# arindamrc/video_analytics

Hardware: AMD Instinct MI355X
Metric: clips/sec (224x224, RGB+10-flow two-stream) (higher is better)
Workload: dtype f32; 1 GPU; two-stream 224x224, 10-frame TV-L1 flow stack (5 scales x 5 warps x 300 its, fixed), VGG-16 spatial+temporal, batch=32 per GPU; global_batch=32, block_iters=0, tvl1_math=exact, flow_streams=2, batches_in_flight=1, tvl1_params=, tvl1_hip_blob=20e9f45376b19dd960a619139aafc0e8722a8659, parallelism=clips sharded x1, finite=True

## Files before the change

video_analytics_amd/csrc/tvl1.hip:

```cpp
#include "va_internal.h"
#include <cmath>
#include <algorithm>
#include <cstdlib>
#include <cstring>
#include <utility>
#include <type_traits>

namespace {

constexpr int kMaxScales = 16;
constexpr int kMaxRadius = 8;
constexpr int kNF_STATE = 6;
constexpr int kNF_RO = 4;

struct Taps {
    float g[2 * kMaxRadius + 1];
    int R;
};

__device__ __forceinline__ int d_min(int a, int b) { return a < b ? a : b; }
__device__ __forceinline__ int d_max(int a, int b) { return a > b ? a : b; }

__device__ __forceinline__ int pslot(int x, int perm) { return perm ? ((x & ~3) | ((x & 1) << 1) | ((x >> 1) & 1)) : x; }

__device__ __forceinline__ float bilinear(const float* __restrict__ img, int w, int h, int pitch, float x, float y, int perm = 0)
{
    x = fminf(fmaxf(x, 0.0f), (float)(w - 1));
    y = fminf(fmaxf(y, 0.0f), (float)(h - 1));
    const int x0 = (int)x, y0 = (int)y;
    const int x1 = d_min(x0 + 1, w - 1), y1 = d_min(y0 + 1, h - 1);
    const float ax = x - (float)x0, ay = y - (float)y0;
    const int s0 = pslot(x0, perm), s1 = pslot(x1, perm);
    const float a = img[y0 * pitch + s0], b = img[y0 * pitch + s1];
    const float c = img[y1 * pitch + s0], d = img[y1 * pitch + s1];
    const float top = fmaf(ax, b - a, a);
    const float bot = fmaf(ax, d - c, c);
    return fmaf(ay, bot - top, top);
}


template <typename T>
__global__ void k_frames_to_level0(const T* __restrict__ frames, float* __restrict__ pyr0, int w, int h, int pitch,
                                   size_t plane)
{
    const int f = blockIdx.y;
    const int idx = blockIdx.x * blockDim.x + threadIdx.x;
    if (idx >= w * h) return;
    const int y = idx / w, x = idx - y * w;
    pyr0[(size_t)f * 3 * plane + (size_t)y * pitch + x] = (float)frames[(size_t)f * w * h + idx];
}

template <bool VERT>
__global__ void k_gauss(const float* __restrict__ src, size_t src_fstride, float* __restrict__ dst, size_t dst_fstride,
                        int w, int h, int pitch, Taps t)
{
    const int f = blockIdx.y;
    const int idx = blockIdx.x * blockDim.x + threadIdx.x;
    if (idx >= w * h) return;
    const int y = idx / w, x = idx - y * w;
    const float* s = src + (size_t)f * src_fstride;
    const int R = t.R;
    float acc;
    if (VERT) {
        acc = t.g[0] * s[d_max(y - R, 0) * pitch + x];
        for (int k = -R + 1; k <= R; ++k) acc = fmaf(t.g[k + R], s[d_min(d_max(y + k, 0), h - 1) * pitch + x], acc);
    } else {
        acc = t.g[0] * s[y * pitch + d_max(x - R, 0)];
// ... 61 lines not shown
    }
    float r[3];
#pragma unroll
    for (int k = 0; k < 3; ++k) {
        const float top = fmaf(ax, b[k] - a[k], a[k]);
        const float bot = fmaf(ax, d[k] - c[k], c[k]);
        r[k] = fmaf(ay, bot - top, top);
    }
    v0 = r[0];
    v1 = r[1];
    v2 = r[2];
}

__global__ void k_warp(const float* __restrict__ pyr, size_t plane, int w, int h, int pitch, int fps,
                       const float* __restrict__ stA, const float* __restrict__ stB, const int* __restrict__ sel, int cur,
                       int* __restrict__ base, float* __restrict__ ro, int pair0, int perm)
{
    unsigned lid = blockIdx.y * gridDim.x + blockIdx.x;
    {
        const unsigned nb = gridDim.x * gridDim.y, q = nb / 8, r = nb % 8, xcd = lid % 8, kk = lid / 8;
        lid = (xcd < r ? xcd * (q + 1) : r * (q + 1) + (xcd - r) * q) + kk;
    }
    const int pair = pair0 + (int)(lid / gridDim.x);
    const int idx = (int)(lid % gridDim.x) * blockDim.x + threadIdx.x;
    const int which = sel ? sel[pair] : cur;
    if (base && idx == 0) base[pair] = which;
    const bool active = idx < w * h;
    const int y = active ? idx / w : 0, x = active ? idx - y * w : 0;
    const int seq = pair / (fps - 1), k = pair - seq * (fps - 1);
    const int f0 = seq * fps + k;
    const float* I0 = pyr + (size_t)f0 * 3 * plane;
    const float* I1 = pyr + (size_t)(f0 + 1) * 3 * plane;
    const float* st = (which ? stB : stA) + (size_t)pair * kNF_STATE * plane;
    const size_t o = (size_t)y * pitch + x, op = (size_t)y * pitch + pslot(x, perm);
    const float u1 = active ? st[op] : 0.0f, u2 = active ? st[plane + op] : 0.0f;
    float Iw, Iwx, Iwy;
    bilinear3_shfl(I1, plane, w, h, pitch, (float)x + u1, (float)y + u2, active, Iw, Iwx, Iwy);
    if (!active) return;
    const float grad = fmaf(Iwy, Iwy, Iwx * Iwx);
    float* r = ro + (size_t)pair * kNF_RO * plane;
    r[op] = Iwx;
    r[plane + op] = Iwy;
    r[2 * plane + op] = fmaf(-Iwy, u2, fmaf(-Iwx, u1, Iw - I0[o]));
    r[3 * plane + op] = grad < 1e-10f ? 0.0f : 1.0f / grad;
}

__global__ void k_upsample(const float* __restrict__ stA, const float* __restrict__ stB, const int* __restrict__ sel,
                           int cur, int cw, int ch, int cpitch, size_t cplane, float* __restrict__ tmp, int fw, int fh,
                           int fpitch, size_t fplane, float inv_step, int cperm)
{
    const int pair = blockIdx.y;
    const int idx = blockIdx.x * blockDim.x + threadIdx.x;
    if (idx >= fw * fh) return;
    const int which = sel ? sel[pair] : cur;
    const float* src = (which ? stB : stA) + (size_t)pair * kNF_STATE * cplane;
    float* dst = tmp + (size_t)pair * 2 * fplane;
    const int y = idx / fw, x = idx - y * fw;
    const float rx = (float)cw / (float)fw, ry = (float)ch / (float)fh;
    const size_t o = (size_t)y * fpitch + x;
    dst[o] = bilinear(src, cw, ch, cpitch, (float)x * rx, (float)y * ry, cperm) * inv_step;
    dst[fplane + o] = bilinear(src + cplane, cw, ch, cpitch, (float)x * rx, (float)y * ry, cperm) * inv_step;
}

__global__ void k_level_init(const float* __restrict__ tmp, float* __restrict__ st0, int w, int h, int pitch, size_t plane, int perm)
{
    const int pair = blockIdx.y;
    const int idx = blockIdx.x * blockDim.x + threadIdx.x;
    if (idx >= pitch * h) return;
    const int y = idx / pitch, x = idx - y * pitch;
    const size_t o = (size_t)y * pitch + x, op = (size_t)y * pitch + pslot(x, perm);
    const float* t = tmp + (size_t)pair * 2 * plane;
    float* dst = st0 + (size_t)pair * kNF_STATE * plane;
    dst[op] = x < w ? t[o] : 0.0f;
    dst[plane + op] = x < w ? t[plane + o] : 0.0f;
    dst[2 * plane + op] = 0.0f;
    dst[3 * plane + op] = 0.0f;
    dst[4 * plane + op] = 0.0f;
    dst[5 * plane + op] = 0.0f;
}

__global__ void k_zero_pad(float* __restrict__ buf, int nf, int w, int h, int pitch, size_t plane, int perm)
{
    const int pair = blockIdx.y, pw = pitch - w;
    const int idx = blockIdx.x * blockDim.x + threadIdx.x;
    if (idx >= pw * h * nf) return;
    const int f = idx / (pw * h), r = idx - f * pw * h, y = r / pw, x = w + r - y * pw;
    buf[((size_t)pair * nf + f) * plane + (size_t)y * pitch + pslot(x, perm)] = 0.0f;
}

__global__ void k_flow_out(const float* __restrict__ stA, const float* __restrict__ stB, const int* __restrict__ sel,
                           int cur, int w, int h, int pitch, size_t plane, float* __restrict__ flow, int perm)
{
    const int pair = blockIdx.y;
    const int idx = blockIdx.x * blockDim.x + threadIdx.x;
    if (idx >= w * h) return;
    const int which = sel ? sel[pair] : cur;
    const float* st = (which ? stB : stA) + (size_t)pair * kNF_STATE * plane;
    const int y = idx / w, x = idx - y * w;
    flow[((size_t)pair * 2) * w * h + idx] = st[(size_t)y * pitch + pslot(x, perm)];
    flow[((size_t)pair * 2 + 1) * w * h + idx] = st[plane + (size_t)y * pitch + pslot(x, perm)];
}

__global__ void k_flow_to_stack(const float* __restrict__ flow, float* __restrict__ stack, size_t n, float bound,
                                float mean, float stdv)
{
    const size_t i = (size_t)blockIdx.x * blockDim.x + threadIdx.x;
    if (i >= n) return;
    const float t = (255.0f * (flow[i] + bound)) / (2.0f * bound);
    const float q = rintf(fminf(fmaxf(t, 0.0f), 255.0f));
    stack[i] = (q / 255.0f - mean) / stdv;
}


struct IterArgs {
    const float* ro;
    const float* stA;
    const float* stB;
    float* outA;
    float* outB;
    const int* base;
    int* sel;
    unsigned long long* err;
    unsigned long long qthr;
    size_t plane;
    int cur;
    int w, h, pitch;
    int K;
    int ntx, nty, HX;
    int it, iters;
    int rev;
    int pair0;
    float l_t, taut, theta;
};

__device__ __forceinline__ float dpp_from_left(float v)
{
    return __builtin_bit_cast(float, __builtin_amdgcn_update_dpp(0, __builtin_bit_cast(int, v), 0x138, 0xf, 0xf, true));
}
__device__ __forceinline__ float dpp_from_right(float v)
{
    return __builtin_bit_cast(float, __builtin_amdgcn_update_dpp(0, __builtin_bit_cast(int, v), 0x130, 0xf, 0xf, true));
}

typedef float f2 __attribute__((ext_vector_type(2)));
#ifndef VA_REV
#define VA_REV 1
#endif
#ifndef VA_STREAM_QUEUE_DEFAULT
#define VA_STREAM_QUEUE_DEFAULT 0
#endif
#ifndef VA_STREAM4_DEFAULT
#define VA_STREAM4_DEFAULT 0
#endif
#ifndef VA_STREAM_UNROLL2
#define VA_STREAM_UNROLL2 1
#endif
#ifndef VA_CHUNK
#define VA_CHUNK 1
#endif
#ifndef VA_TIMING_SKIP
#define VA_TIMING_SKIP 0
#endif
#ifndef VA_CHUNK_MB
#define VA_CHUNK_MB 150.0
#endif

__device__ __forceinline__ f2 pk_fma(f2 a, f2 b, f2 c) { return __builtin_elementwise_fma(a, b, c); }
__device__ __forceinline__ float sub_s(float a, float b)
{
    float r;
    asm("v_sub_f32 %0, %1, %2" : "=v"(r) : "v"(a), "v"(b));
    return r;
}
__device__ __forceinline__ f2 splat(float v) { return f2{v, v}; }

constexpr float kSqrtReg = 7.888609052210118e-31f;
__device__ __forceinline__ f2 sqrt_exact_pk(f2 s)
// ... 449 lines not shown
    typedef StreamShape<KH, NCH> SH;
    constexpr int NP = R::NP, NT = R::NT, SW = 64 * PPL, KC = SH::KC;
    constexpr int NRING = stream_ring_rows<KH, NWV, NCH>() > 0 ? stream_ring_rows<KH, NWV, NCH>() : 1;
    __shared__ f2 ringP_[SUBS][NRING][kNF_RO][NP][64];
    __shared__ float ringT_[SUBS][NRING][kNF_RO][NT ? 64 : 1];
    __shared__ f2 ifaceP_[SUBS][NWV > 1 ? NWV - 1 : 1][2][kNF_STATE][NP][64];
    __shared__ float ifaceT_[SUBS][NWV > 1 ? NWV - 1 : 1][2][kNF_STATE][NT ? 64 : 1];
    auto& ringP = ringP_[sub];
    auto& ringT = ringT_[sub];
    auto& ifaceP = ifaceP_[sub];
    auto& ifaceT = ifaceT_[sub];

    const int sx = job % a.nsx, ch = job / a.nsx;
    const int w = a.w, h = a.h, pitch = a.pitch;
    const int lane = threadIdx.x & 63;
    const int wv = NWV == 1 ? 0 : role >= 0 ? role : __builtin_amdgcn_readfirstlane((int)(threadIdx.x >> 6));
    const int ox = sx * (SW - 2 * a.HX);
    const int vx0 = ox + (sx > 0 ? a.HX : 0), vx1 = (sx == a.nsx - 1) ? pitch : ox + SW - a.HX;
    const int x0 = ox + PPL * (half ? (lane & 31) : lane);
    const bool colok = x0 < pitch && !(half == 2 && lane >= 32);
    const bool stok = colok && x0 >= vx0 && x0 < vx1;
    const int a0 = ch * a.R, b0 = d_min(h, a0 + a.R);
    const int ys = d_max(0, a0 - K), ye = d_min(h, b0 + K);

    const int planeb = (int)(a.plane * sizeof(float)), pitchb = pitch * (int)sizeof(float);
    const int npr = half == 1 ? 2 : 1;
    const __amdgpu_buffer_rsrc_t rs_ro = __builtin_amdgcn_make_buffer_rsrc(
        const_cast<float*>(a.ro + (size_t)pair * kNF_RO * a.plane), 0, npr * kNF_RO * planeb, 0x00020000);
    const __amdgpu_buffer_rsrc_t rs_in = __builtin_amdgcn_make_buffer_rsrc(
        const_cast<float*>(sin_all + (size_t)pair * kNF_STATE * a.plane), 0, npr * kNF_STATE * planeb, 0x00020000);
    const __amdgpu_buffer_rsrc_t rs_out = __builtin_amdgcn_make_buffer_rsrc(sout_all + (size_t)pair * kNF_STATE * a.plane, 0,
                                                                           npr * kNF_STATE * planeb, 0x00020000);
    const bool second = half == 1 && lane >= 32;
    const int loff = colok ? x0 * (int)sizeof(float) + (second ? kNF_STATE * planeb : 0) : 0;
    const int loff_ro = colok ? x0 * (int)sizeof(float) + (second ? kNF_RO * planeb : 0) : 0;

    R mx;
    mx.t = 0.0f;
#pragma clang loop unroll(full)
    for (int i = 0; i < PPL; ++i) row_set(mx, i, x0 + i < w - 1 ? 1.0f : 0.0f);
    const float l_t = a.l_t, taut = a.taut, theta = a.theta;
    const R zero = row_splat<PPL>(0.0f), one = row_splat<PPL>(1.0f);

    auto ring_put = [&](int slot, int f, const R& v) __attribute__((always_inline)) {
#pragma clang loop unroll(full)
        for (int j = 0; j < NP; ++j) ringP[slot][f][j][lane] = v.p[j];
        if constexpr (NT) ringT[slot][f][lane] = v.t;
    };
    auto ring_get = [&](int slot, int f) __attribute__((always_inline)) -> R {
        R v;
#pragma clang loop unroll(full)
        for (int j = 0; j < NP; ++j) v.p[j] = ringP[slot][f][j][lane];
        v.t = 0.0f;
        if constexpr (NT) v.t = ringT[slot][f][lane];
        return v;
    };
    auto if_put = [&](int wb, int b, int f, const R& v) __attribute__((always_inline)) {
#pragma clang loop unroll(full)
        for (int j = 0; j < NP; ++j) ifaceP[wb][b][f][j][lane] = v.p[j];
        if constexpr (NT) ifaceT[wb][b][f][lane] = v.t;
    };
    auto if_get = [&](int wb, int b, int f) __attribute__((always_inline)) -> R {
        R v;
#pragma clang loop unroll(full)
        for (int j = 0; j < NP; ++j) v.p[j] = ifaceP[wb][b][f][j][lane];
        v.t = 0.0f;
        if constexpr (NT) v.t = ifaceT[wb][b][f][lane];
        return v;
    };

    for (int r = wv; r < NRING; r += NWV)
#pragma clang loop unroll(full)
        for (int f = 0; f < kNF_RO; ++f) ring_put(r, f, zero);
    if constexpr (NWV > 1) {
        if (wv < NWV - 1)
#pragma clang loop unroll(full)
            for (int f = 0; f < kNF_STATE; ++f) {
                if_put(wv, 0, f, zero);
                if_put(wv, 1, f, zero);
            }
        __syncthreads();
    }

    auto ld = [&](const __amdgpu_buffer_rsrc_t& r, int f, int y) -> R { return row_load<PPL>(r, loff, f * planeb + y * pitchb); };
    auto ld_ro = [&](int f, int y) -> R { return row_load<PPL>(rs_ro, loff_ro, f * planeb + y * pitchb); };
    auto st = [&](const R& v, int f, int y) { row_store<PPL>(v, rs_out, loff, f * planeb + y * pitchb); };

    const int nsteps = active ? b0 - ys + K + (NWV * NCH - 1) : 0;

    auto run = [&](auto wave_tag) __attribute__((always_inline)) {
        constexpr int W = decltype(wave_tag)::value;
        constexpr bool FIRST = W == 0, LAST = W == NWV - 1;
        constexpr int G0 = W * KH, LAG = W * SH::SPAN;

        R P11[KH], P12[KH], P21[KH], P22[KH], U1[KH], U2[KH];
#pragma clang loop unroll(full)
        for (int t = 0; t < KH; ++t) P11[t] = P12[t] = P21[t] = P22[t] = U1[t] = U2[t] = zero;
        SR latch[NCH > 1 ? NCH - 1 : 1];
#pragma clang loop unroll(full)
        for (int c = 0; c < (NCH > 1 ? NCH - 1 : 1); ++c) latch[c] = SR{zero, zero, zero, zero, zero, zero};
        R nst[kNF_STATE], nro[kNF_RO], rprev[kNF_RO] = {zero, zero, zero, zero};
        constexpr bool KEEP = LAST && stream_keep_last<KH, NWV, NCH>();
        R keep[kNF_RO] = {zero, zero, zero, zero};
#pragma clang loop unroll(full)
        for (int f = 0; f < kNF_STATE; ++f) nst[f] = FIRST ? ld(rs_in, f, ys) : zero;
#pragma clang loop unroll(full)
        for (int f = 0; f < kNF_RO; ++f) nro[f] = FIRST ? ld_ro(f, ys) : zero;

        auto level = [&](int t, SR& c, const R& wx, const R& wy, const R& rc, const R& ig, const float my, auto my1_tag) __attribute__((always_inline)) {
            constexpr bool MY1 = decltype(my1_tag)::value;
            const R dx11 = r_diff_back(c.p11), dx21 = r_diff_back(c.p21);
            const R div1 = r_add(dx11, r_sub(c.p12, P12[t]));
            const R div2 = r_add(dx21, r_sub(c.p22, P22[t]));
            const R rho = r_fma(wy, c.u2, r_fma(wx, c.u1, rc));
            const R tt = r_negmul(rho, ig);
            const R fi = r_med3(tt, -l_t, l_t);
            const R v1 = r_fma(fi, wx, c.u1);
            const R v2 = r_fma(fi, wy, c.u2);
            const R n1 = r_fma_s(theta, div1, v1);
            const R n2 = r_fma_s(theta, div2, v2);
            const R d1x = r_diff_fwd(U1[t]), d2x = r_diff_fwd(U2[t]);
            const R u1x = r_mul(d1x, mx), u1y = MY1 ? r_sub(n1, U1[t]) : r_mul_s(r_sub(n1, U1[t]), my);
            const R u2x = r_mul(d2x, mx), u2y = MY1 ? r_sub(n2, U2[t]) : r_mul_s(r_sub(n2, U2[t]), my);
            const R s1 = r_fma(u1y, u1y, r_fma_c(u1x, u1x, kSqrtReg));
            const R s2 = r_fma(u2y, u2y, r_fma_c(u2x, u2x, kSqrtReg));
            const R d1 = r_fma_s(taut, r_sqrt<PPL, FAST>(s1), one);
            const R d2 = r_fma_s(taut, r_sqrt<PPL, FAST>(s2), one);
            R q1, q2;
            if constexpr (FAST) {
                q1 = r_rcp<PPL, true>(d1);
                q2 = r_rcp<PPL, true>(d2);
            } else {
                const R rinv = r_rcp<PPL, false>(r_mul(d1, d2));
                q1 = r_mul(d2, rinv);
                q2 = r_mul(d1, rinv);
            }
            const R o11 = r_mul(r_fma_s(taut, u1x, P11[t]), q1);
            const R o12 = r_mul(r_fma_s(taut, u1y, P12[t]), q1);
            const R o21 = r_mul(r_fma_s(taut, u2x, P21[t]), q2);
            const R o22 = r_mul(r_fma_s(taut, u2y, P22[t]), q2);
            const R ou1 = U1[t], ou2 = U2[t];
            P11[t] = c.p11;
            P12[t] = c.p12;
            P21[t] = c.p21;
            P22[t] = c.p22;
            U1[t] = n1;
            U2[t] = n2;
            c.u1 = ou1;
            c.u2 = ou2;
            c.p11 = o11;
            c.p12 = o12;
            c.p21 = o21;
            c.p22 = o22;
        };

        auto step = [&](const int s, auto steady_tag) __attribute__((always_inline)) {
            constexpr bool STEADY = decltype(steady_tag)::value;
            const int s0 = s % NRING;
            SR cc[NCH];
            R r0[kNF_RO] = {zero, zero, zero, zero};
            if constexpr (FIRST) {
                cc[0] = SR{nst[0], nst[1], nst[2], nst[3], nst[4], nst[5]};
#pragma clang loop unroll(full)
                for (int f = 0; f < kNF_RO; ++f) r0[f] = nro[f];
                const int rn = d_min(ys + s + 1, ye - 1);
                if (!(STEADY && (VA_TIMING_SKIP & 2))) {
#pragma clang loop unroll(full)
                    for (int f = 0; f < kNF_STATE; ++f) nst[f] = ld(rs_in, f, rn);
#pragma clang loop unroll(full)
                    for (int f = 0; f < kNF_RO; ++f) nro[f] = ld_ro(f, rn);
                }
                if constexpr (NWV > 1) {
                    const int sl = s0 == 0 ? NRING - 1 : s0 - 1;
                    if (!(STEADY && (VA_TIMING_SKIP & 32)))
#pragma clang loop unroll(full)
                        for (int f = 0; f < kNF_RO; ++f) ring_put(sl, f, rprev[f]);
                }
                if (!(VA_TIMING_SKIP & 16)) __builtin_amdgcn_sched_barrier(0);
            } else {
                const int bsel = (s + 1) & 1;
                if (STEADY && (VA_TIMING_SKIP & 4)) {
                    cc[0] = SR{U1[0], U2[0], P11[0], P12[0], P21[0], P22[0]};
                } else {
                    cc[0].u1 = if_get(W - 1, bsel, 0);
                    cc[0].u2 = if_get(W - 1, bsel, 1);
                    cc[0].p11 = if_get(W - 1, bsel, 2);
                    cc[0].p12 = if_get(W - 1, bsel, 3);
                    cc[0].p21 = if_get(W - 1, bsel, 4);
                    cc[0].p22 = if_get(W - 1, bsel, 5);
                }
            }
#pragma clang loop unroll(full)
            for (int c = 1; c < NCH; ++c) cc[c] = latch[c - 1];
            auto slot_of = [&](int t) {
                const int c = (LAG + SH::lpos(t)) % NRING;
                return s0 - c < 0 ? s0 - c + NRING : s0 - c;
            };
            if constexpr (STEADY) {
                R q[NCH][kNF_RO];
#pragma clang loop unroll(full)
                for (int c = 0; c < NCH; ++c) {
                    if (FIRST && c == 0) {
#pragma clang loop unroll(full)
// ... 38 lines not shown
                    for (int c = 0; c < NCH; ++c)
#pragma clang loop unroll(full)
                        for (int f = 0; f < kNF_RO; ++f) q[c][f] = nq[c][f];
                }
            } else {
#pragma clang loop unroll(full)
                for (int t = 0; t < KH; ++t) {
                    const int g = G0 + t, rin = ys + s - LAG - SH::lpos(t);
                    const int lo = d_max(0, a0 - (K - g)), hi = d_min(h, b0 + (K - g) - 1);
                    const bool act = g < K && rin >= lo && rin <= hi;
                    if (act) {
                        const float my = rin - 1 < h - 1 ? 1.0f : 0.0f;
                        if (FIRST && t == 0) {
                            level(0, cc[0], r0[0], r0[1], r0[2], r0[3], my, std::false_type{});
                        } else if (KEEP && t == KH - 1) {
                            level(t, cc[t / KC], keep[0], keep[1], keep[2], keep[3], my, std::false_type{});
                        } else {
                            const int slot = slot_of(t);
                            level(t, cc[t / KC], ring_get(slot, 0), ring_get(slot, 1), ring_get(slot, 2), ring_get(slot, 3), my, std::false_type{});
                        }
                    }
                }
                if constexpr (KEEP) {
                    const int slot = slot_of(KH - 2);
#pragma clang loop unroll(full)
                    for (int f = 0; f < kNF_RO; ++f) keep[f] = ring_get(slot, f);
                }
            }
#pragma clang loop unroll(full)
            for (int c = 0; c + 1 < NCH; ++c) latch[c] = cc[c];
            const SR& co = cc[NCH - 1];
            if constexpr (LAST) {
                const int rout = ys + s - K - (NWV * NCH - 1);
                if (stok && rout >= a0 && rout < b0 && !(STEADY && (VA_TIMING_SKIP & 1))) {
                    st(co.u1, 0, rout);
                    st(co.u2, 1, rout);
                    st(co.p11, 2, rout);
                    st(co.p12, 3, rout);
                    st(co.p21, 4, rout);
                    st(co.p22, 5, rout);
                }
            } else {
                const int bsel = s & 1;
                if (!(STEADY && (VA_TIMING_SKIP & 4))) {
                    if_put(W, bsel, 0, co.u1);
                    if_put(W, bsel, 1, co.u2);
                    if_put(W, bsel, 2, co.p11);
                    if_put(W, bsel, 3, co.p12);
                    if_put(W, bsel, 4, co.p21);
                    if_put(W, bsel, 5, co.p22);
                }
            }
            if constexpr (FIRST) {
                if constexpr (NWV == 1) {
#pragma clang loop unroll(full)
                    for (int f = 0; f < kNF_RO; ++f) ring_put(s0, f, r0[f]);
                } else {
#pragma clang loop unroll(full)
                    for (int f = 0; f < kNF_RO; ++f) rprev[f] = r0[f];
                }
            }
            if constexpr (NWV > 1) asm volatile("s_waitcnt lgkmcnt(0)\n\ts_barrier" ::: "memory");
        };
        int s_a = 0, s_b = nsteps;
#pragma clang loop unroll(full)
        for (int t = 0; t < KH; ++t) {
            const int g = G0 + t, p = LAG + SH::lpos(t) - ys;
            s_a = d_max(s_a, d_max(0, a0 - (K - g)) + p);
            s_b = d_min(s_b, d_min(h - 1, d_min(h, b0 + (K - g) - 1)) + p + 1);
        }
        if (K < G0 + KH || s_a > s_b || !active) s_a = s_b = 0;
        int s = 0;
        for (; s < s_a; ++s) step(s, std::false_type{});
#if VA_STREAM_UNROLL2
        if constexpr (NWV > 1 || KH > 10)
            for (; s + 1 < s_b; s += 2) {
                step(s, std::true_type{});
                step(s + 1, std::true_type{});
            }
#endif
        for (; s < s_b; ++s) step(s, std::true_type{});
        for (; s < nsteps; ++s) step(s, std::false_type{});
        if constexpr (SUBS > 1)
            for (; s < steps_pad; ++s) asm volatile("s_waitcnt lgkmcnt(0)\n\ts_barrier" ::: "memory");
    };
    if constexpr (NWV == 1) {
        run(std::integral_constant<int, 0>{});
    } else if constexpr (NWV == 2) {
        if (wv == 0) run(std::integral_constant<int, 0>{});
        else run(std::integral_constant<int, NWV - 1>{});
    } else if constexpr (NWV == 3) {
        if (wv == 0) run(std::integral_constant<int, 0>{});
        else if (wv == 1) run(std::integral_constant<int, 1>{});
        else run(std::integral_constant<int, 2>{});
    } else {
        static_assert(NWV == 4, "pipelines of one to four waves");
        if (wv == 0) run(std::integral_constant<int, 0>{});
        else if (wv == 1) run(std::integral_constant<int, 1>{});
        else if (wv == 2) run(std::integral_constant<int, 2>{});
        else run(std::integral_constant<int, 3>{});
    }
}

template <int PPL, int KH, int NWV, bool FAST, int NCH = 1>
__global__ void __launch_bounds__(NWV * 64)
    __attribute__((amdgpu_waves_per_eu((NWV == 1 && KH > 10) ? 1 : 2, (NWV == 1 && KH > 10) ? 1 : NWV >= 3 ? 4 : 2)))
    k_iter_stream(StreamArgs a)
{
    unsigned lid = blockIdx.y * gridDim.x + blockIdx.x;
    {
        const unsigned nb = gridDim.x * gridDim.y, q = nb / 8, r = nb % 8, xcd = lid % 8, kk = lid / 8;
        lid = (xcd < r ? xcd * (q + 1) : r * (q + 1) + (xcd - r) * q) + kk;
// ... 231 lines not shown
    return (nwv * kh + nwv) * kNF_RO * ppl * 256 + (nwv > 1 ? nwv - 1 : 1) * 2 * (kNF_STATE * ppl * 256 + 4);
}
constexpr int kRowsLdsMax = 160 * 1024 - 512;
#endif
bool pick_rows(const va_tvl1_params* p, int h, int pitch, RowsPick& rp)
{
#ifndef VA_EXPERIMENTS
    (void)p, (void)h, (void)pitch, (void)rp;
    return false;
#else
    int nwv = kRowsShapes[0][0], kh = kRowsShapes[0][1];
    if (p->tuning[VA_TUNE_ROWS_CFG] > 0) {
        nwv = p->tuning[VA_TUNE_ROWS_CFG] >> 4;
        kh = p->tuning[VA_TUNE_ROWS_CFG] & 15;
    }
    bool known = false;
    for (int i = 0; i < kNumRowsShapes; ++i) known = known || (kRowsShapes[i][0] == nwv && kRowsShapes[i][1] == kh);
    if (!known) return false;
    rp.ppl = pitch <= 128 ? 2 : pitch <= 192 ? 3 : 4;
    if (pitch > 256) return false;
    rp.nwv = nwv;
    rp.kh = kh;
    if (rows_lds_bytes(rp.ppl, nwv, kh) > kRowsLdsMax) return false;
    const int Kfull = nwv * kh;
    rp.K = p->iters < Kfull ? p->iters : Kfull;
    rp.N = va_cdiv(p->iters, rp.K);
    rp.K0 = p->iters - (rp.N - 1) * rp.K;
    if (rp.N >= 2047 || pitch % rp.ppl != 0) return false;
    return h >= Kfull + nwv + 4 && h < (1 << kRowIdRowBits);
#endif
}

enum { LK_TILE = 0, LK_STREAM = 1, LK_ROWS = 2 };
bool level_streams(const va_tvl1_params* p, bool eps, int s, int w, int h, size_t plane);
int level_kernel(const va_tvl1_params* p, bool eps, int s, int w, int h, int pitch, size_t plane, RowsPick* rp)
{
    RowsPick tmp{};
    if (!rp) rp = &tmp;
    if (eps || (double)plane * kNF_STATE * sizeof(float) >= 2147483648.0) return LK_TILE;
    const bool rows_ok = pick_rows(p, h, pitch, *rp);
    if (p->tile_mask & kRowsBit) return rows_ok ? LK_ROWS : LK_STREAM;
    if ((p->tile_mask & ~kNoNarrowBit) != 0) return level_streams(p, eps, s, w, h, plane) ? LK_STREAM : LK_TILE;
    if (p->tuning[VA_TUNE_ROWS_LEVELS] >= 0 || p->tuning[VA_TUNE_STREAM_LEVELS] >= 0) {
        if (p->tuning[VA_TUNE_ROWS_LEVELS] >= 0 && ((p->tuning[VA_TUNE_ROWS_LEVELS] >> s) & 1) && rows_ok) return LK_ROWS;
        return p->tuning[VA_TUNE_STREAM_LEVELS] >= 0 && ((p->tuning[VA_TUNE_STREAM_LEVELS] >> s) & 1) ? LK_STREAM : LK_TILE;
    }
    return level_streams(p, eps, s, w, h, plane) ? LK_STREAM : LK_TILE;
}

#ifdef VA_EXPERIMENTS
template <int PPL, bool FAST>
int launch_rows(const RowsPick& rp, const RowsArgs& a, int npairs, hipStream_t st)
{
#define VA_ROWS_CASE(NWV_, KH_)                                                           \
    if constexpr (rows_lds_bytes(PPL, NWV_, KH_) <= kRowsLdsMax) {                        \
        if (rp.nwv == NWV_ && rp.kh == KH_) {                                             \
            k_iter_rows<PPL, KH_, NWV_, FAST><<<npairs, NWV_ * 64, 0, st>>>(a);           \
            return VA_OK;                                                                 \
        }                                                                                 \
    }
    VA_ROWS_CASE(4, 4)
    VA_ROWS_CASE(2, 8)
    VA_ROWS_CASE(3, 5)
    VA_ROWS_CASE(4, 3)
    VA_ROWS_CASE(8, 2)
    VA_ROWS_CASE(2, 6)
// ... 53 lines not shown
        sum += g[k + R];
    }
    for (int k = 0; k <= 2 * R; ++k) t->g[k] = (float)(g[k] / sum);
    t->R = R;
    return R;
}

int check_params(const va_tvl1_params* p, int w, int h, int n_seq, int fps)
{
    VA_CHECK_ARG(p != nullptr, "va_tvl1: params is NULL");
    VA_CHECK_ARG(w >= 16 && h >= 16 && w <= 16384 && h <= 16384, "va_tvl1: frame size %dx%d out of range [16,16384]", w, h);
    VA_CHECK_ARG(n_seq >= 1 && fps >= 2, "va_tvl1: need n_seq >= 1 and frames_per_seq >= 2 (got %d, %d)", n_seq, fps);
    VA_CHECK_ARG((long)n_seq * (fps - 1) <= 65535, "va_tvl1: more than 65535 pairs in one call");
    VA_CHECK_ARG(p->nscales >= 1 && p->warps >= 1 && p->iters >= 1, "va_tvl1: nscales, warps, iters must be >= 1");
    VA_CHECK_ARG(p->scale_step > 0.0f && p->scale_step < 1.0f, "va_tvl1: scale_step must be in (0,1)");
    VA_CHECK_ARG(p->tau > 0.0f && p->lambda > 0.0f && p->theta > 0.0f, "va_tvl1: tau, lambda, theta must be > 0");
    VA_CHECK_ARG(p->block_iters >= 0 && p->block_iters <= 64, "va_tvl1: block_iters must be in [0,64]");
    VA_CHECK_ARG(p->fast_math == 0 || p->fast_math == 1, "va_tvl1: fast_math must be 0 or 1");
    VA_CHECK_ARG(p->tile_mask >= 0 && p->tile_mask < (1 << (kNumCfgs + 3)), "va_tvl1: tile_mask must be in [0, %d]", (1 << (kNumCfgs + 3)) - 1);
    VA_CHECK_ARG(p->tuning[VA_TUNE_ROWS_LEVELS] >= -1 && p->tuning[VA_TUNE_ROWS_LEVELS] < (1 << kMaxScales) && p->tuning[VA_TUNE_ROWS_CFG] >= 0 && p->tuning[VA_TUNE_ROWS_CFG] < 256,
                 "va_tvl1: rows_levels must be -1 or a level bit set, rows_cfg in [0,255]");
    VA_CHECK_ARG(p->tuning[VA_TUNE_STREAM_PPL] == 0 || p->tuning[VA_TUNE_STREAM_PPL] == 2 || p->tuning[VA_TUNE_STREAM_PPL] == 3, "va_tvl1: stream_ppl must be 0 (default), 2 or 3");
    VA_CHECK_ARG(p->tuning[VA_TUNE_STREAM_QUEUE] >= 0 && p->tuning[VA_TUNE_STREAM_QUEUE] <= 2, "va_tvl1: stream_queue must be 0 (default), 1 (queued) or 2 (a launch per pass)");
    VA_CHECK_ARG(p->tuning[VA_TUNE_STREAM_LEVELS] >= -1 && p->tuning[VA_TUNE_STREAM_LEVELS] < (1 << kMaxScales) && (p->tuning[VA_TUNE_STREAM_WAVES] >= 0 && p->tuning[VA_TUNE_STREAM_WAVES] < kMwFirst + kNumMwShapes) &&
                     p->tuning[VA_TUNE_STREAM_CHUNKS] >= 0 && p->tuning[VA_TUNE_STREAM_SLOTS] >= 0,
                 "va_tvl1: stream_levels must be -1 or a level bit set, stream_waves in [0, 12], stream_chunks and stream_slots >= 0");
    VA_CHECK_ARG(p->tau / p->theta <= 1000.0f && p->lambda * p->theta <= 1000.0f, "va_tvl1: tau/theta and lambda*theta must be <= 1000");
    VA_CHECK_ARG(!(p->tuning[VA_TUNE_STREAM_WAVES] == 3 && p->fast_math), "va_tvl1: stream_waves = 3 (one deep wave) is compiled for the exact arithmetic only");
    if (!kVaExperiments) {
        const int sw = p->tuning[VA_TUNE_STREAM_WAVES];
        VA_CHECK_ARG(sw != 3 && sw != 4 && sw != 5 && sw != 6 && sw <= kMwFirst + 2 && p->tuning[VA_TUNE_STREAM_PPL] != 3 && p->tuning[VA_TUNE_STREAM_QUEUE] != 1 &&
                         p->tuning[VA_TUNE_ROWS_LEVELS] <= 0 && p->tuning[VA_TUNE_ROWS_CFG] == 0 && !(p->tile_mask & kRowsBit),
                     "va_tvl1: this tuning value selects an experiment kernel (k_iter_rows, k_iter_stream_q, k_iter_stream4, one deep "
                     "wave, two chains per wave, four waves x four levels, 3 pixels per lane); build the library with -DVA_EXPERIMENTS (make EXPERIMENTS=1) to get them");
    }
    return VA_OK;
}

int pyramid_sizes(int w, int h, const va_tvl1_params* p, int* ws, int* hs)
{
    int n = 1;
    ws[0] = w;
    hs[0] = h;
    const int want = p->nscales > kMaxScales ? kMaxScales : p->nscales;
    while (n < want) {
        const int nw = (int)((float)ws[n - 1] * p->scale_step + 0.5f);
        const int nh = (int)((float)hs[n - 1] * p->scale_step + 0.5f);
        if ((nw < nh ? nw : nh) < 16) break;
        ws[n] = nw;
        hs[n] = nh;
        ++n;
    }
    return n;
}

void make_plan(Plan& P, int w, int h, int n_seq, int fps, const va_tvl1_params* p)
{
    P.ns = pyramid_sizes(w, h, p, P.ws, P.hs);
    P.F = fps;
    P.NF = n_seq * fps;
    P.NP = n_seq * (fps - 1);
    size_t off = 0;
    for (int s = 0; s < P.ns; ++s) {
        P.lk[s] = plan_level(p, s, P.ws[s], P.hs[s], &P.pitch[s], &P.plane[s], &P.rows[s]);
        P.off_pyr[s] = off;
        off += va_align_up((size_t)P.NF * 3 * P.plane[s] * sizeof(float), 256);
    }
// ... 156 lines not shown
        k_gauss<false><<<g, TPB, 0, st>>>(pyr[s - 1], 3 * P.plane[s - 1], tmp1, P.plane_max, pw, ph, pp, taps);
        k_gauss<true><<<g, TPB, 0, st>>>(tmp1, P.plane_max, tmp2, P.plane_max, pw, ph, pp, taps);
        const dim3 g2(va_cdiv(P.ws[s] * P.hs[s], TPB), P.NF);
        k_resample<<<g2, TPB, 0, st>>>(tmp2, P.plane_max, pw, ph, pp, pyr[s], 3 * P.plane[s], P.ws[s], P.hs[s], P.pitch[s]);
        VA_LAUNCH_CHECK();
    }
    for (int s = 0; s < P.ns; ++s) {
        const dim3 g(va_cdiv(P.ws[s] * P.hs[s], TPB), P.NF);
        k_grad<<<g, TPB, 0, st>>>(pyr[s], P.ws[s], P.hs[s], P.pitch[s], P.plane[s]);
        VA_LAUNCH_CHECK();
    }

    const int sc = P.ns - 1;
    VA_HIP(hipMemsetAsync(state[0], 0, (size_t)P.NP * kNF_STATE * P.plane[sc] * sizeof(float), st));
    VA_HIP(hipMemsetAsync(sel, 0, (size_t)P.NP * 2 * sizeof(int), st));
    int cur = 0;
    int K0 = p->block_iters;
    if (eps) K0 = 1;

    for (int s = sc; s >= 0; --s) {
        const int lw = P.ws[s], lh = P.hs[s], lp = P.pitch[s];
        const size_t plane = P.plane[s];
        const unsigned tmask = (unsigned)p->tile_mask & (unsigned)(kStreamBit - 1);
        const TilePick tp = K0 > 0 ? pick_tiles(lw, lh, K0, tmask) : pick_tiles_auto(lw, lh, p->iters, tmask);
        const RowsPick rp = P.rows[s];
        const int lk = P.lk[s];
        const size_t st_lo = state[0] < state[1] ? 0 : 1;
        const size_t st_span = (size_t)((char*)state[st_lo ^ 1] - (char*)state[st_lo]) + (size_t)kNF_STATE * plane * sizeof(float);
        if (lk == LK_ROWS && st_span >= 2147483648ull) {
            va_set_error("va_tvl1_flow: internal error: state buffers too far apart for k_iter_rows");
            return VA_ERR_INVALID;
        }
        const bool strm = lk == LK_STREAM, rows = lk == LK_ROWS;
        const int perm = (strm || rows) ? 0 : 1;
        if (lp != lw) {
            k_zero_pad<<<dim3(va_cdiv((lp - lw) * lh * kNF_RO, TPB), P.NP), TPB, 0, st>>>(ro, kNF_RO, lw, lh, lp, plane, perm);
            VA_LAUNCH_CHECK();
        }
        const int cp = (eps || !VA_CHUNK || strm || rows) ? P.NP : chunk_pairs(lw, lh, tp, P.NP);
        const int cur_in = cur;
        for (int c0 = 0; c0 < P.NP; c0 += cp) {
        const int nc = P.NP - c0 < cp ? P.NP - c0 : cp;
        const dim3 gpc(va_cdiv(lw * lh, TPB), nc);
        cur = cur_in;
        for (int wp = 0; wp < p->warps; ++wp) {
            k_warp<<<gpc, TPB, 0, st>>>(pyr[s], plane, lw, lh, lp, P.F, state[0], state[1], eps ? sel : nullptr, cur,
                                         eps ? base : nullptr, ro, c0, perm);
            VA_LAUNCH_CHECK();
            if (eps) VA_HIP(hipMemsetAsync(err, 0, (size_t)P.NP * p->iters * sizeof(unsigned long long), st));
            va_prof_span span{};
            if (ctx->prof_on) {
                span = prof_get(ctx);
                span.level = s;
                VA_HIP(hipEventRecord(span.beg, st));
            }
            IterArgs a{};
            a.ro = ro;
            a.stA = state[0];
            a.stB = state[1];
            a.outA = state[0];
            a.outB = state[1];
            a.base = base;
            a.sel = sel;
            a.err = err;
            a.qthr = eps ? (unsigned long long)((double)p->epsilon * (double)p->epsilon * (double)lw * (double)lh * 4294967296.0) : 0ull;
            a.plane = plane;
            a.w = lw;
// ... 153 lines not shown
                a.cur = cur;
                a.K = tk.K;
                a.it = it;
                a.rev = VA_REV ? (launches & 1) : 0;
                if (eps) {
                    if (p->fast_math) launch_iter<true, true>(tk, a, nc, st);
                    else launch_iter<true, false>(tk, a, nc, st);
                } else {
                    if (p->fast_math) launch_iter<false, true>(tk, a, nc, st);
                    else launch_iter<false, false>(tk, a, nc, st);
                }
                cur ^= 1;
                it += tk.K;
                ++launches;
            }
            VA_LAUNCH_CHECK();
            if (ctx->prof_on) {
                VA_HIP(hipEventRecord(span.end, st));
                ctx->prof_spans.push_back(span);
                ctx->prof_launches += launches;
                ctx->prof_pxiters += (double)nc * lw * lh * p->iters;
                ctx->prof_pxwarps += (double)nc * lw * lh;
                if (s < kVaProfLevels) {
                    ctx->prof_level_pxiters[s] += (double)nc * lw * lh * p->iters;
                    ctx->prof_level_launches[s] += launches;
                }
            }
        }
        }
        if (s > 0) {
            const dim3 g(va_cdiv(P.ws[s - 1] * P.hs[s - 1], TPB), P.NP);
            k_upsample<<<g, TPB, 0, st>>>(state[0], state[1], eps ? sel : nullptr, cur, lw, lh, lp, plane, ro, P.ws[s - 1],
                                           P.hs[s - 1], P.pitch[s - 1], P.plane[s - 1], 1.0f / p->scale_step, perm);
            const int fperm = P.lk[s - 1] != LK_TILE ? 0 : 1;
            const dim3 gi(va_cdiv(P.pitch[s - 1] * P.hs[s - 1], TPB), P.NP);
            k_level_init<<<gi, TPB, 0, st>>>(ro, state[0], P.ws[s - 1], P.hs[s - 1], P.pitch[s - 1], P.plane[s - 1], fperm);
            VA_LAUNCH_CHECK();
            cur = 0;
            if (eps) VA_HIP(hipMemsetAsync(sel, 0, (size_t)P.NP * sizeof(int), st));
        }
    }
    {
        const dim3 g(va_cdiv(w * h, TPB), P.NP);
        k_flow_out<<<g, TPB, 0, st>>>(state[0], state[1], eps ? sel : nullptr, cur, w, h, P.pitch[0], P.plane[0], (float*)flow,
                                       P.lk[0] != LK_TILE ? 0 : 1);
        VA_LAUNCH_CHECK();
    }
    return VA_OK;
}

extern "C" int va_flow_to_stack(va_ctx* ctx, const void* flow, int n_pairs, int w, int h, float bound, float mean,
                                float stdv, void* stack, void* stream)
{
    VA_CHECK_ARG(ctx != nullptr, "va_flow_to_stack: ctx is NULL");
    VA_USE_DEVICE(ctx);
    VA_CHECK_ARG(flow != nullptr && stack != nullptr, "va_flow_to_stack: NULL buffer");
    VA_CHECK_ARG(n_pairs >= 1 && w >= 1 && h >= 1, "va_flow_to_stack: bad shape");
    VA_CHECK_ARG(bound > 0.0f && stdv > 0.0f, "va_flow_to_stack: bound and std must be > 0");
    const size_t n = (size_t)n_pairs * 2 * w * h;
    k_flow_to_stack<<<(unsigned)((n + 255) / 256), 256, 0, (hipStream_t)stream>>>((const float*)flow, (float*)stack, n, bound, mean, stdv);
    VA_LAUNCH_CHECK();
    return VA_OK;
}

extern "C" int va_selftest_exact_math(va_ctx* ctx, float lo, float hi, unsigned long long* mismatches, void* stream)
{
    VA_CHECK_ARG(ctx != nullptr && mismatches != nullptr, "va_selftest_exact_math: NULL argument");
    VA_USE_DEVICE(ctx);
    VA_CHECK_ARG(lo >= kSqrtReg && hi <= 1e30f && lo <= hi, "va_selftest_exact_math: range must lie in [2^-100, 1e30]");
    unsigned ulo, uhi;
    memcpy(&ulo, &lo, 4);
    memcpy(&uhi, &hi, 4);
    VA_HIP(hipMemsetAsync(mismatches, 0, 2 * sizeof(unsigned long long), (hipStream_t)stream));
    k_selftest_exact_math<<<4096, 256, 0, (hipStream_t)stream>>>(ulo, (unsigned long long)uhi - ulo + 1, mismatches);
    VA_LAUNCH_CHECK();
    return VA_OK;
}

// ... 67 lines not shown
```

Measured before the change: 258.7 clips/s.

## Interleave TV-L1 state planes in pairs for 128-bit row loads in stream kernel

Adds a PERM_PAIRS layout where pairs of state/ro field planes (u1/u2, p11/p12, p21/p22, Iwx/Iwy, ...) are interleaved per row in 2-pixel groups. The streaming iteration kernel with 2 pixels per lane can then load and store two fields with one 16-byte buffer access instead of two 8-byte ones, cutting memory instruction count. All helper kernels (warp, upsample, level_init, zero_pad, flow_out) are updated to index through a shared fslot helper. A peeled extra steady step is also added for some configurations. The risk is extra index arithmetic in the helper kernels and layout mismatches between levels.

```diff
diff --git a/video_analytics_amd/csrc/tvl1.hip b/video_analytics_amd/csrc/tvl1.hip
--- a/video_analytics_amd/csrc/tvl1.hip
+++ b/video_analytics_amd/csrc/tvl1.hip
@@ -23,16 +23,39 @@
 
 __device__ __forceinline__ int pslot(int x, int perm) { return perm ? ((x & ~3) | ((x & 1) << 1) | ((x >> 1) & 1)) : x; }
 
-__device__ __forceinline__ float bilinear(const float* __restrict__ img, int w, int h, int pitch, float x, float y, int perm = 0)
+#ifndef VA_STATE_PAIRS
+#define VA_STATE_PAIRS 1
+#endif
+enum { PERM_PLAIN = 0, PERM_TILE = 1, PERM_PAIRS = 2 };
+__device__ __forceinline__ size_t fslot(int f, int y, int x, int pitch, size_t plane, int perm)
+{
+    if (perm == PERM_PAIRS) return (size_t)(f >> 1) * 2 * plane + (size_t)y * 2 * pitch + (((x & ~1) << 1) | ((f & 1) << 1) | (x & 1));
+    return (size_t)f * plane + (size_t)y * pitch + pslot(x, perm);
+}
+
+__device__ __forceinline__ float bilinear(const float* __restrict__ img, int w, int h, int pitch, float x, float y)
 {
     x = fminf(fmaxf(x, 0.0f), (float)(w - 1));
     y = fminf(fmaxf(y, 0.0f), (float)(h - 1));
     const int x0 = (int)x, y0 = (int)y;
     const int x1 = d_min(x0 + 1, w - 1), y1 = d_min(y0 + 1, h - 1);
     const float ax = x - (float)x0, ay = y - (float)y0;
-    const int s0 = pslot(x0, perm), s1 = pslot(x1, perm);
-    const float a = img[y0 * pitch + s0], b = img[y0 * pitch + s1];
-    const float c = img[y1 * pitch + s0], d = img[y1 * pitch + s1];
+    const float a = img[y0 * pitch + x0], b = img[y0 * pitch + x1];
+    const float c = img[y1 * pitch + x0], d = img[y1 * pitch + x1];
+    const float top = fmaf(ax, b - a, a);
+    const float bot = fmaf(ax, d - c, c);
+    return fmaf(ay, bot - top, top);
+}
+__device__ __forceinline__ float bilinear_state(const float* __restrict__ st, int f, size_t plane, int w, int h, int pitch, float x,
+                                                float y, int perm)
+{
+    x = fminf(fmaxf(x, 0.0f), (float)(w - 1));
+    y = fminf(fmaxf(y, 0.0f), (float)(h - 1));
+    const int x0 = (int)x, y0 = (int)y;
+    const int x1 = d_min(x0 + 1, w - 1), y1 = d_min(y0 + 1, h - 1);
+    const float ax = x - (float)x0, ay = y - (float)y0;
+    const float a = st[fslot(f, y0, x0, pitch, plane, perm)], b = st[fslot(f, y0, x1, pitch, plane, perm)];
+    const float c = st[fslot(f, y1, x0, pitch, plane, perm)], d = st[fslot(f, y1, x1, pitch, plane, perm)];
     const float top = fmaf(ax, b - a, a);
     const float bot = fmaf(ax, d - c, c);
     return fmaf(ay, bot - top, top);
@@ -160,17 +183,17 @@
     const float* I0 = pyr + (size_t)f0 * 3 * plane;
     const float* I1 = pyr + (size_t)(f0 + 1) * 3 * plane;
     const float* st = (which ? stB : stA) + (size_t)pair * kNF_STATE * plane;
-    const size_t o = (size_t)y * pitch + x, op = (size_t)y * pitch + pslot(x, perm);
-    const float u1 = active ? st[op] : 0.0f, u2 = active ? st[plane + op] : 0.0f;
+    const size_t o = (size_t)y * pitch + x;
+    const float u1 = active ? st[fslot(0, y, x, pitch, plane, perm)] : 0.0f, u2 = active ? st[fslot(1, y, x, pitch, plane, perm)] : 0.0f;
     float Iw, Iwx, Iwy;
     bilinear3_shfl(I1, plane, w, h, pitch, (float)x + u1, (float)y + u2, active, Iw, Iwx, Iwy);
     if (!active) return;
     const float grad = fmaf(Iwy, Iwy, Iwx * Iwx);
     float* r = ro + (size_t)pair * kNF_RO * plane;
-    r[op] = Iwx;
-    r[plane + op] = Iwy;
-    r[2 * plane + op] = fmaf(-Iwy, u2, fmaf(-Iwx, u1, Iw - I0[o]));
-    r[3 * plane + op] = grad < 1e-10f ? 0.0f : 1.0f / grad;
+    r[fslot(0, y, x, pitch, plane, perm)] = Iwx;
+    r[fslot(1, y, x, pitch, plane, perm)] = Iwy;
+    r[fslot(2, y, x, pitch, plane, perm)] = fmaf(-Iwy, u2, fmaf(-Iwx, u1, Iw - I0[o]));
+    r[fslot(3, y, x, pitch, plane, perm)] = grad < 1e-10f ? 0.0f : 1.0f / grad;
 }
 
 __global__ void k_upsample(const float* __restrict__ stA, const float* __restrict__ stB, const int* __restrict__ sel,
@@ -186,8 +209,8 @@
     const int y = idx / fw, x = idx - y * fw;
     const float rx = (float)cw / (float)fw, ry = (float)ch / (float)fh;
     const size_t o = (size_t)y * fpitch + x;
-    dst[o] = bilinear(src, cw, ch, cpitch, (float)x * rx, (float)y * ry, cperm) * inv_step;
-    dst[fplane + o] = bilinear(src + cplane, cw, ch, cpitch, (float)x * rx, (float)y * ry, cperm) * inv_step;
+    dst[o] = bilinear_state(src, 0, cplane, cw, ch, cpitch, (float)x * rx, (float)y * ry, cperm) * inv_step;
+    dst[fplane + o] = bilinear_state(src, 1, cplane, cw, ch, cpitch, (float)x * rx, (float)y * ry, cperm) * inv_step;
 }
 
 __global__ void k_level_init(const float* __restrict__ tmp, float* __restrict__ st0, int w, int h, int pitch, size_t plane, int perm)
@@ -196,15 +219,13 @@
     const int idx = blockIdx.x * blockDim.x + threadIdx.x;
     if (idx >= pitch * h) return;
     const int y = idx / pitch, x = idx - y * pitch;
-    const size_t o = (size_t)y * pitch + x, op = (size_t)y * pitch + pslot(x, perm);
+    const size_t o = (size_t)y * pitch + x;
     const float* t = tmp + (size_t)pair * 2 * plane;
     float* dst = st0 + (size_t)pair * kNF_STATE * plane;
-    dst[op] = x < w ? t[o] : 0.0f;
-    dst[plane + op] = x < w ? t[plane + o] : 0.0f;
-    dst[2 * plane + op] = 0.0f;
-    dst[3 * plane + op] = 0.0f;
-    dst[4 * plane + op] = 0.0f;
-    dst[5 * plane + op] = 0.0f;
+    dst[fslot(0, y, x, pitch, plane, perm)] = x < w ? t[o] : 0.0f;
+    dst[fslot(1, y, x, pitch, plane, perm)] = x < w ? t[plane + o] : 0.0f;
+#pragma unroll
+    for (int f = 2; f < kNF_STATE; ++f) dst[fslot(f, y, x, pitch, plane, perm)] = 0.0f;
 }
 
 __global__ void k_zero_pad(float* __restrict__ buf, int nf, int w, int h, int pitch, size_t plane, int perm)
@@ -213,7 +234,7 @@
     const int idx = blockIdx.x * blockDim.x + threadIdx.x;
     if (idx >= pw * h * nf) return;
     const int f = idx / (pw * h), r = idx - f * pw * h, y = r / pw, x = w + r - y * pw;
-    buf[((size_t)pair * nf + f) * plane + (size_t)y * pitch + pslot(x, perm)] = 0.0f;
+    buf[(size_t)pair * nf * plane + fslot(f, y, x, pitch, plane, perm)] = 0.0f;
 }
 
 __global__ void k_flow_out(const float* __restrict__ stA, const float* __restrict__ stB, const int* __restrict__ sel,
@@ -225,8 +246,8 @@
     const int which = sel ? sel[pair] : cur;
     const float* st = (which ? stB : stA) + (size_t)pair * kNF_STATE * plane;
     const int y = idx / w, x = idx - y * w;
-    flow[((size_t)pair * 2) * w * h + idx] = st[(size_t)y * pitch + pslot(x, perm)];
-    flow[((size_t)pair * 2 + 1) * w * h + idx] = st[plane + (size_t)y * pitch + pslot(x, perm)];
+    flow[((size_t)pair * 2) * w * h + idx] = st[fslot(0, y, x, pitch, plane, perm)];
+    flow[((size_t)pair * 2 + 1) * w * h + idx] = st[fslot(1, y, x, pitch, plane, perm)];
 }
 
 __global__ void k_flow_to_stack(const float* __restrict__ flow, float* __restrict__ stack, size_t n, float bound,
@@ -271,6 +292,7 @@
 }
 
 typedef float f2 __attribute__((ext_vector_type(2)));
+typedef float f4 __attribute__((ext_vector_type(4)));
 #ifndef VA_REV
 #define VA_REV 1
 #endif
@@ -786,8 +808,10 @@
     const __amdgpu_buffer_rsrc_t rs_out = __builtin_amdgcn_make_buffer_rsrc(sout_all + (size_t)pair * kNF_STATE * a.plane, 0,
                                                                            npr * kNF_STATE * planeb, 0x00020000);
     const bool second = half == 1 && lane >= 32;
-    const int loff = colok ? x0 * (int)sizeof(float) + (second ? kNF_STATE * planeb : 0) : 0;
-    const int loff_ro = colok ? x0 * (int)sizeof(float) + (second ? kNF_RO * planeb : 0) : 0;
+    constexpr bool PAIRS = VA_STATE_PAIRS && PPL == 2;
+    constexpr int LB = (PAIRS ? 2 : 1) * (int)sizeof(float);
+    const int loff = colok ? x0 * LB + (second ? kNF_STATE * planeb : 0) : 0;
+    const int loff_ro = colok ? x0 * LB + (second ? kNF_RO * planeb : 0) : 0;
 
     R mx;
     mx.t = 0.0f;
@@ -836,9 +860,41 @@
         __syncthreads();
     }
 
-    auto ld = [&](const __amdgpu_buffer_rsrc_t& r, int f, int y) -> R { return row_load<PPL>(r, loff, f * planeb + y * pitchb); };
-    auto ld_ro = [&](int f, int y) -> R { return row_load<PPL>(rs_ro, loff_ro, f * planeb + y * pitchb); };
-    auto st = [&](const R& v, int f, int y) { row_store<PPL>(v, rs_out, loff, f * planeb + y * pitchb); };
+    auto ld_row = [&](const __amdgpu_buffer_rsrc_t& r, int lo, int y, auto nf_tag, R* o) __attribute__((always_inline)) {
+        constexpr int NF = decltype(nf_tag)::value;
+        if constexpr (PAIRS) {
+#pragma clang loop unroll(full)
+            for (int k = 0; k < NF / 2; ++k) {
+                const f4 v = __builtin_bit_cast(f4, RowIo<4>::ld(r, lo, (k * planeb + y * pitchb) * 2));
+                o[2 * k].p[0] = __builtin_shufflevector(v, v, 0, 1);
+                o[2 * k + 1].p[0] = __builtin_shufflevector(v, v, 2, 3);
+                o[2 * k].t = o[2 * k + 1].t = 0.0f;
+            }
+        } else {
+#pragma clang loop unroll(full)
+            for (int f = 0; f < NF; ++f) o[f] = row_load<PPL>(r, lo, f * planeb + y * pitchb);
+        }
+    };
+    auto st_row = [&](const SR& c, int y) __attribute__((always_inline)) {
+        if constexpr (PAIRS) {
+            const R* a[3] = {&c.u1, &c.p11, &c.p21};
+            const R* b[3] = {&c.u2, &c.p12, &c.p22};
+#pragma clang loop unroll(full)
+            for (int k = 0; k < 3; ++k) {
+                const f4 v = __builtin_shufflevector(a[k]->p[0], b[k]->p[0], 0, 1, 2, 3);
+                RowIo<4>::st(__builtin_bit_cast(typename RowIo<4>::V, v), rs_out, loff, (k * planeb + y * pitchb) * 2);
+            }
+        } else {
+            row_store<PPL>(c.u1, rs_out, loff, 0 * planeb + y * pitchb);
+            row_store<PPL>(c.u2, rs_out, loff, 1 * planeb + y * pitchb);
+            row_store<PPL>(c.p11, rs_out, loff, 2 * planeb + y * pitchb);
+            row_store<PPL>(c.p12, rs_out, loff, 3 * planeb + y * pitchb);
+            row_store<PPL>(c.p21, rs_out, loff, 4 * planeb + y * pitchb);
+            row_store<PPL>(c.p22, rs_out, loff, 5 * planeb + y * pitchb);
+        }
+    };
+    constexpr std::integral_constant<int, kNF_STATE> nf_state{};
+    constexpr std::integral_constant<int, kNF_RO> nf_ro{};
 
     const int nsteps = active ? b0 - ys + K + (NWV * NCH - 1) : 0;
 
@@ -857,9 +913,13 @@
         constexpr bool KEEP = LAST && stream_keep_last<KH, NWV, NCH>();
         R keep[kNF_RO] = {zero, zero, zero, zero};
 #pragma clang loop unroll(full)
-        for (int f = 0; f < kNF_STATE; ++f) nst[f] = FIRST ? ld(rs_in, f, ys) : zero;
-#pragma clang loop unroll(full)
-        for (int f = 0; f < kNF_RO; ++f) nro[f] = FIRST ? ld_ro(f, ys) : zero;
+        for (int f = 0; f < kNF_STATE; ++f) nst[f] = zero;
+#pragma clang loop unroll(full)
+        for (int f = 0; f < kNF_RO; ++f) nro[f] = zero;
+        if constexpr (FIRST) {
+            ld_row(rs_in, loff, ys, nf_state, nst);
+            ld_row(rs_ro, loff_ro, ys, nf_ro, nro);
+        }
 
         auto level = [&](int t, SR& c, const R& wx, const R& wy, const R& rc, const R& ig, const float my, auto my1_tag) __attribute__((always_inline)) {
             constexpr bool MY1 = decltype(my1_tag)::value;
@@ -919,10 +979,8 @@
                 for (int f = 0; f < kNF_RO; ++f) r0[f] = nro[f];
                 const int rn = d_min(ys + s + 1, ye - 1);
                 if (!(STEADY && (VA_TIMING_SKIP & 2))) {
-#pragma clang loop unroll(full)
-                    for (int f = 0; f < kNF_STATE; ++f) nst[f] = ld(rs_in, f, rn);
-#pragma clang loop unroll(full)
-                    for (int f = 0; f < kNF_RO; ++f) nro[f] = ld_ro(f, rn);
+                    ld_row(rs_in, loff, rn, nf_state, nst);
+                    ld_row(rs_ro, loff_ro, rn, nf_ro, nro);
                 }
                 if constexpr (NWV > 1) {
                     const int sl = s0 == 0 ? NRING - 1 : s0 - 1;
@@ -1027,14 +1085,7 @@
             const SR& co = cc[NCH - 1];
             if constexpr (LAST) {
                 const int rout = ys + s - K - (NWV * NCH - 1);
-                if (stok && rout >= a0 && rout < b0 && !(STEADY && (VA_TIMING_SKIP & 1))) {
-                    st(co.u1, 0, rout);
-                    st(co.u2, 1, rout);
-                    st(co.p11, 2, rout);
-                    st(co.p12, 3, rout);
-                    st(co.p21, 4, rout);
-                    st(co.p22, 5, rout);
-                }
+                if (stok && rout >= a0 && rout < b0 && !(STEADY && (VA_TIMING_SKIP & 1))) st_row(co, rout);
             } else {
                 const int bsel = s & 1;
                 if (!(STEADY && (VA_TIMING_SKIP & 4))) {
@@ -1073,6 +1124,9 @@
                 step(s, std::true_type{});
                 step(s + 1, std::true_type{});
             }
+        if constexpr (NWV > 1 || KH > 10) {
+            if (s < s_b) step(s++, std::true_type{});
+        } else
 #endif
         for (; s < s_b; ++s) step(s, std::true_type{});
         for (; s < nsteps; ++s) step(s, std::false_type{});
@@ -1370,6 +1424,11 @@
 }
 
 enum { LK_TILE = 0, LK_STREAM = 1, LK_ROWS = 2 };
+int level_perm(const va_tvl1_params* p, int lk, int w)
+{
+    if (lk == LK_TILE) return PERM_TILE;
+    return lk == LK_STREAM && VA_STATE_PAIRS && stream_ppl(p, w) == 2 ? PERM_PAIRS : PERM_PLAIN;
+}
 bool level_streams(const va_tvl1_params* p, bool eps, int s, int w, int h, size_t plane);
 int level_kernel(const va_tvl1_params* p, bool eps, int s, int w, int h, int pitch, size_t plane, RowsPick* rp)
 {
@@ -1489,7 +1548,8 @@
         VA_CHECK_ARG(sw != 3 && sw != 4 && sw != 5 && sw != 6 && sw <= kMwFirst + 2 && p->tuning[VA_TUNE_STREAM_PPL] != 3 && p->tuning[VA_TUNE_STREAM_QUEUE] != 1 &&
                          p->tuning[VA_TUNE_ROWS_LEVELS] <= 0 && p->tuning[VA_TUNE_ROWS_CFG] == 0 && !(p->tile_mask & kRowsBit),
                      "va_tvl1: this tuning value selects an experiment kernel (k_iter_rows, k_iter_stream_q, k_iter_stream4, one deep "
-                     "wave, two chains per wave, four waves x four levels, 3 pixels per lane); build the library with -DVA_EXPERIMENTS (make EXPERIMENTS=1) to get them");
+                     "wave, two chains per wave, three waves x five or six levels, four waves x six levels, 3 pixels per lane); build the "
+                     "library with -DVA_EXPERIMENTS (make EXPERIMENTS=1) to get them");
     }
     return VA_OK;
 }
@@ -1712,7 +1772,7 @@
             return VA_ERR_INVALID;
         }
         const bool strm = lk == LK_STREAM, rows = lk == LK_ROWS;
-        const int perm = (strm || rows) ? 0 : 1;
+        const int perm = level_perm(p, lk, lw);
         if (lp != lw) {
             k_zero_pad<<<dim3(va_cdiv((lp - lw) * lh * kNF_RO, TPB), P.NP), TPB, 0, st>>>(ro, kNF_RO, lw, lh, lp, plane, perm);
             VA_LAUNCH_CHECK();
@@ -1932,7 +1992,7 @@
             const dim3 g(va_cdiv(P.ws[s - 1] * P.hs[s - 1], TPB), P.NP);
             k_upsample<<<g, TPB, 0, st>>>(state[0], state[1], eps ? sel : nullptr, cur, lw, lh, lp, plane, ro, P.ws[s - 1],
                                            P.hs[s - 1], P.pitch[s - 1], P.plane[s - 1], 1.0f / p->scale_step, perm);
-            const int fperm = P.lk[s - 1] != LK_TILE ? 0 : 1;
+            const int fperm = level_perm(p, P.lk[s - 1], P.ws[s - 1]);
             const dim3 gi(va_cdiv(P.pitch[s - 1] * P.hs[s - 1], TPB), P.NP);
             k_level_init<<<gi, TPB, 0, st>>>(ro, state[0], P.ws[s - 1], P.hs[s - 1], P.pitch[s - 1], P.plane[s - 1], fperm);
             VA_LAUNCH_CHECK();
@@ -1943,7 +2003,7 @@
     {
         const dim3 g(va_cdiv(w * h, TPB), P.NP);
         k_flow_out<<<g, TPB, 0, st>>>(state[0], state[1], eps ? sel : nullptr, cur, w, h, P.pitch[0], P.plane[0], (float*)flow,
-                                       P.lk[0] != LK_TILE ? 0 : 1);
+                                       level_perm(p, P.lk[0], w));
         VA_LAUNCH_CHECK();
     }
     return VA_OK;
```

Result: no change. 260.2 clips/s, median of 6 (+0.6%).
